# OPPO-Mente-Lab/PEA-Diffusion

Measured on AMD Instinct MI355X. Metric: training images/sec (SDXL 1024px bf16, adapter-only bwd), higher is better.
Workload: dtype bf16

## Files before the change

### include/pea_hip.h

```cpp
#ifndef PEA_HIP_H
#define PEA_HIP_H
#include <stdint.h>
#ifdef __cplusplus
extern "C" {
#endif

#define PEA_OK 0
#define PEA_E_INVALID (-1)
#define PEA_E_HIP (-2)
#define PEA_E_SHAPE (-3)
#define PEA_E_STATE (-4)
#define PEA_E_NOTFOUND (-5)
#define PEA_E_TIMEOUT (-6)

const char* pea_last_error(void);
int pea_version(void);
int pea_device_count(void);


int pea_op_gemm(const void* A, int lda, const void* W, int ldw, void* C, int ldc, int M, int N, int K, float alpha,
                const float* bias, const void* rowvec, int ldrv, int rows_per_batch, int act, void* preact,
                int ldpre, const void* res, int ldres, int out_f32, int accum_f32, void* stream);

int pea_op_gemm_qscale(const void* A, int lda, const void* W, int ldw, void* C, int ldc, int M, int N, int K, const float* bias,
// ... 176 lines not shown
int pea_unet_residual_info(void* unet, int i, int* C, int* H, int* W);
int pea_unet_set_residuals(void* unet, int n, const void* const* ptrs, int dtype, float scale, void* stream);
int pea_unet_set_inpaint_cond(void* unet, const float* mask, const float* masked_latents, int cond_batch, int latent_batch,
                              void* stream);
int pea_unet_clear_inpaint_cond(void* unet);
int pea_unet_set_freeu(void* unet, float s1, float s2, float b1, float b2, void* stream);
int pea_unet_clear_freeu(void* unet);
int pea_unet_ip_plan(const pea_unet_config* cfg, int n_tokens, int* n_layers, int* cols, long long* n_params);
int pea_unet_ip_create(void* unet, int n_tokens);
int pea_unet_ip_load_weight(void* unet, const char* key, const float* src, long long numel, void* stream);
int pea_unet_ip_set_tokens(void* unet, const float* tokens, void* stream);
int pea_unet_ip_set_scale(void* unet, float scale);
int pea_unet_ip_clear(void* unet);
int pea_unet_ip_destroy(void* unet);
int pea_unet_ip_export_kv(void* unet, float* out, long long* rows, int* cols, void* stream);
int pea_unet_ip_create_sets(void* unet, int n_sets, const int* n_tokens);
int pea_unet_ip_load_weight_set(void* unet, int set, const char* key, const float* src, long long numel, void* stream);
int pea_unet_ip_set_tokens_set(void* unet, int set, const float* tokens, void* stream);
int pea_unet_ip_set_scale_set(void* unet, int set, float scale);
int pea_unet_ip_clear_set(void* unet, int set);
int pea_unet_ip_set_layer_scales(void* unet, int set, const float* scales, int n_layers);
int pea_unet_ip_query_counts(void* unet, int* counts, int cap, int* n);
int pea_unet_ip_set_mask(void* unet, int set, int Sq, const float* mask, int Bm, void* stream);
int pea_unet_destroy(void* unet);

int pea_controlnet_create(const pea_unet_config* cfg, int B, int H, int W, int L, void** out);
int pea_controlnet_set_cond(void* cn, const float* image, void* stream);
int pea_controlnet_forward(void* cn, const float* x, const float* t, const void* ehs, int ehs_dtype, const void* text,
                           int text_dtype, const float* time_ids, void* stream);
int pea_controlnet_num_outputs(void* cn);
int pea_controlnet_output(void* cn, int i, void** ptr, int* C, int* H, int* W);
int pea_controlnet_export_nchw(void* cn, int i, float* dst, void* stream);

typedef struct pea_text_config {
  int vocab, max_pos, width, heads, layers, intermediate;
  int act;
  int flavor;
  int proj_dim;
  float eps;
  int pos_offset;
  long long eos_id;
  int rel_buckets;
  int rel_max_dist;
} pea_text_config;
int pea_text_create(const pea_text_config* cfg, int B, int L, void** out);
int pea_text_plan_attention(const pea_text_config* cfg, int B, int L, int* n_attn, int* n_prescaled);
int pea_text_forward(void* enc, const long long* ids, int hidden_index, float* hidden_out, float* pooled_out, void* stream);
int pea_text_rel_bias(void* enc, float* bias_out, void* stream);

typedef struct pea_vision_config {
  int image_size, patch_size, width, heads, layers, intermediate;
  int act;
  int proj_dim;
  float eps;
} pea_vision_config;
int pea_vision_create(const pea_vision_config* cfg, int B, void** out);
int pea_vision_plan(const pea_vision_config* cfg, int B, long long* n_params, int* n_tokens, int* n_attn);
int pea_vision_forward(void* enc, const float* pixels, int hidden_index, float* hidden_out, float* pooled_out, float* embeds_out,
                       void* stream);
typedef struct pea_resampler_config {
  int embed_dim, dim, heads, depth, n_queries, ff_inner, out_dim;
  float eps;
} pea_resampler_config;
int pea_resampler_create(const pea_resampler_config* cfg, int B, int S, void** out);
int pea_resampler_plan(const pea_resampler_config* cfg, int B, int S, long long* n_params, int* n_attn, int* n_prescaled);
int pea_resampler_plan_weight(const pea_resampler_config* cfg, int B, int S, int i, char* name, int name_len, long long* numel,
                              int* kind, int* d0, int* d1);
int pea_resampler_forward(void* resampler, const float* hidden, float* tokens_out, void* stream);
int pea_op_preprocess(const float* images, int B, int H, int W, float lo, float hi, int quantize, const int* y_first,
                      const int* y_count, const float* y_weights, int y_taps, const int* x_first, const int* x_count,
                      const float* x_weights, int x_taps, int size, int tile_h, int tile_w, int win_h, int win_w, float mean0,
                      float mean1, float mean2, float std0, float std1, float std2, float* out, void* stream);
int pea_op_patchify(const float* pixels, void* rows, int B, int S, int P, int kpad, void* stream);
int pea_op_clip_score(const float* image_embeds, const float* text_embeds, float* out, int B, int D, float w, int clamp,
                      void* stream);

int pea_vae_encoder_create(const pea_unet_config* cfg, int B, int H, int W, void** out);
int pea_vae_latent_shape(void* vae, int* C, int* H, int* W);
int pea_vae_encode(void* vae, const float* pixels, const float* noise, float scaling, float* moments, float* latents,
                   void* stream);
int pea_vae_decoder_create(const pea_unet_config* cfg, int B, int H, int W, void** out);
int pea_vae_decode(void* vae, const float* latents, float inv_scaling, float* image, void* stream);
int pea_unet_num_weights(void* unet);
int pea_unet_weight_info(void* unet, int i, char* name, int name_len, long long* numel, int* kind, int* d0, int* d1);
int pea_unet_load_weight(void* unet, const char* name, const float* src, long long numel, void* stream);
int pea_unet_load_weight_lora(void* unet, const char* name, const float* base, long long numel, int n_adapters,
                              const float* const* downs, const float* const* ups, const int* ranks, const float* scales,
                              void* stream);
int pea_unet_init_random(void* unet, unsigned long long seed, void* stream);
int pea_unet_share_weights(void* dst, void* src);
int pea_unet_forward(void* unet, const float* x, const float* t, const void* ehs, int ehs_dtype, const void* text,
                     int text_dtype, const float* time_ids, float* eps_out, void* stream);
int pea_unet_num_taps(void* unet);
int pea_unet_tap_name(void* unet, int k, char* name, int name_len);
int pea_unet_tap_info(void* unet, int k, void** data, void** grad, int* B, int* H, int* W, int* C);
int pea_unet_tap_export_nchw(void* unet, int k, int grad, float* out, void* stream);
int pea_unet_tap_layout(void* unet, int k);
int pea_unet_tap_import_grad_nchw(void* unet, int k, const float* src, void* stream);
int pea_unet_backward(void* unet, const float* deps, unsigned tap_seed_mask, void* stream);
int pea_unet_input_grads(void* unet, void** d_ehs, void** d_text);
int pea_unet_stacked_grad(void* unet, int which, float* out, long long* rows, int* cols, void* stream);
int pea_unet_stacked_layout(void* unet, int which, int i, char* name, int name_len, int* col_off, int* cols);
int pea_unet_memory(void* unet, long long* weight_bytes, long long* act_bytes, long long* grad_bytes, int* n_ops);
int pea_unet_release_activations(void* unet);

int pea_adapter_create(int in_dim, int out_dim, int hidden_dim, int out_dim1, int use_residual, void** out);
int pea_adapter_destroy(void* ad);
long long pea_adapter_num_params(void* ad);
int pea_adapter_bind(void* ad, float* flat_params);
int pea_adapter_prepare(void* ad, int batch, int L);
int pea_adapter_sync(void* ad, void* stream);
int pea_adapter_forward(void* ad, const void* enc, int dtype, float* pooled, float* tokens, void* stream);
int pea_adapter_backward(void* ad, const float* d_pooled, const float* d_tokens, float* grads, int accumulate,
                         void* stream);

int pea_trainer_create(void* adapter, void* student, void* teacher, float feat_weight, int nan_guard,
                       const float* alphas_cumprod, void** out);
int pea_trainer_destroy(void* tr);
int pea_train_step(void* tr, const float* latents, const float* noise, const long long* timesteps,
                   const float* enc, const float* enc_uncond, const unsigned char* prompt_mask,
                   const long long* zh_or_not, const float* teacher_ehs, const float* teacher_neg,
                   const float* teacher_pooled, const float* time_ids, float grad_scale, float* grads,
                   int accumulate, float* losses, void* stream);
int pea_trainer_set_option(void* tr, const char* name, int value);
int pea_trainer_backward_context(void* trainer, void** unet);
int pea_trainer_get_option(void* trainer, const char* name);
int pea_trainer_release_activations(void* trainer);
int pea_trainer_export(void* tr, int which, float* out, void* stream);

int pea_comm_unique_id(void* out128);
int pea_comm_init(int rank, int world, const void* unique_id128, void** comm_out);
int pea_comm_init_timeout(int rank, int world, const void* unique_id128, double timeout_s, void** comm_out);
int pea_comm_destroy(void* comm);
int pea_comm_world(void* comm);
int pea_comm_rank(void* comm);
int pea_allreduce_grads(void* comm, float* grads, long long n, void* compute_stream);
int pea_comm_join(void* comm, void* stream);
int pea_comm_last_ms(void* comm, float* ms);
int pea_comm_last_exposed_ms(void* comm, float* ms);
int pea_comm_broadcast(void* comm, float* buf, long long n, int root, void* stream);

void pea_prof_enable(int on);
void pea_prof_reset(void);
const char* pea_prof_family_name(int fam);
int pea_prof_dump(const char* path);
int pea_prof_report(int fam, double* ms, double* flops, double* bytes, long long* launches);
int pea_probe_mfma_peak(double seconds, int shape32, double* tflops, double* clock_mhz, void* stream);

void pea_debug_set_attn_tr(int v);
void pea_debug_set_attn_fused_bwd(int v);
void pea_debug_set_attn_xattn(int v);
void pea_debug_set_xattn_bwd_v2(int v);
void pea_debug_set_geglu_bwd_fused(int v);
void pea_debug_set_gemm_variant(int v);
int pea_debug_gemm_dispatch(int M, int N, int K, int mode, int rows_per_batch, int features, int cus, int forced);
int pea_debug_attn_dispatch(const int* q, int* out);
void pea_debug_set_gemm_debug(int v);
void pea_debug_set_gemm_prefetch(const void* p, long long bytes);

int pea_op_attention_fwd_regions(const void* Q, int ldq, const void* K, int ldk, const void* V, int ldv, void* O, int ldo, int B, int H,
                                 int Sq, int R, int Lr, const float* w, int Bw, float scale, int q_prescaled, void* stream);
int pea_unet_set_prompt_regions(void* unet, int R, int Sq, const float* w, int Bw, void* stream);
int pea_unet_clear_prompt_regions(void* unet);
int pea_debug_attn_regions_dispatch(const int* q, int* out);

int pea_op_attention_maps(const void* Q, int ldq, const void* K, int ldk, float* maps, int B, int H, int Sq, int Skv, float scale,
                          int q_prescaled, const int* kv_len, int accumulate, void* stream);
int pea_unet_enable_attention_maps(void* unet, const float* layer_on, int n_layers);
int pea_unet_reset_attention_maps(void* unet, void* stream);
int pea_unet_disable_attention_maps(void* unet);
int pea_unet_attention_maps(void* unet, int Sq, float** maps, long long* n_accumulated);
int pea_debug_attn_maps_dispatch(const int* q, int* out);

int pea_op_attention_fwd_edit(const void* Q, int ldq, const void* K, int ldk, const void* V, int ldv, void* O, int ldo, int B, int H,
                              int Sq, int Skv, const int* src, const void* Mt, int ldm, const float* c, const float* d, float scale,
                              int q_prescaled, void* stream);
int pea_unet_set_prompt_edit(void* unet, const int* src, const void* Mt, const float* cd, int T, int self_until, int self_max_tokens,
                             void* stream);
int pea_unet_set_prompt_edit_step(void* unet, int step);
int pea_unet_clear_prompt_edit(void* unet);
int pea_debug_attn_edit_dispatch(const int* q, int* out);

long long pea_op_attn_adain_scratch_bytes(int B, int H, int S);
int pea_op_attn_adain_coef(const void* Q, int ldq, const void* K, int ldk, int B, int H, int S, const int* ref, float scale,
                           int q_prescaled, int adain_queries, int adain_keys, float* coef, void* scratch, void* stream);
int pea_op_attention_fwd_shared(const void* Q, int ldq, const void* K, int ldk, const void* V, int ldv, void* O, int ldo, int B, int H,
                                int Sq, int Skv, const int* ref, const float* coef, float scale, int q_prescaled,
                                float shared_score_scale, float shared_score_shift, int nd, void* stream);
int pea_unet_set_style_aligned(void* unet, const int* ref, const float* layer_on, int n_layers, int adain_queries, int adain_keys,
                               float shared_score_scale, float shared_score_shift, void* stream);
int pea_unet_clear_style_aligned(void* unet);
int pea_unet_num_self_attention_layers(void* unet);
int pea_debug_attn_shared_dispatch(const int* q, int* out);

int pea_op_attention_colsum_groups(int B, int H, int Sq, int Skv);
int pea_op_attention_colsum(const void* Q, int ldq, const void* K, int ldk, const float* lse, float* part, int B, int H, int Sq, int Skv,
                            float scale, int q_prescaled, void* stream);
int pea_debug_attn_colsum_dispatch(const int* q, int* out);
int pea_op_sag_degrade(const float* latents, const float* eps, const float* part, int G, int map_h, int map_w, const int* iy,
                       const int* ix, float* out, int B, int C, int H, int W, float c_x, float c_e, float o_b, float o_e, void* stream);
int pea_op_cfg_sag_combine(const float* eps, const float* eps_deg, float* out, int B, long long per, int cfg, float guidance_scale,
                           float sag_scale, void* stream);
int pea_unet_enable_sag(void* unet, int layer, int first_sample, int n_samples);
int pea_unet_disable_sag(void* unet);
int pea_unet_sag_colsum(void* unet, float** part, int* G, int* S);

int pea_op_query_blur(void* Q, int ld, int col0, int n, int h, int w, int C, const float* Mh, const float* Mw, void* stream);
int pea_op_query_blur_lds_bytes(int h, int w);
int pea_op_attn_identity(const void* V, int ldv, int col0, void* O, int ldo, long long rows, int C, void* stream);
int pea_op_cfg_pag_combine(const float* eps, float* out, int B, long long per, int cfg, float guidance_scale, float pag_scale,
                           float guidance_rescale, void* workspace, void* stream);
int pea_unet_set_attn_perturb(void* unet, int mode, int first_sample, const float* layer_on, int n_layers, int n_grids,
                              const int* grid_h, const int* grid_w, const float* tables, void* stream);
int pea_unet_clear_attn_perturb(void* unet);

#ifdef __cplusplus
}
#endif
#endif
```

### pea_diffusion_amd/csrc/norm.hip

```cpp
#include "pea_kernels.h"
#ifndef PEA_LN_WT
#define PEA_LN_WT 1
#endif

#define GN_MAX_GROUPS 64

template <int BWD>
__global__ void gn_stats_kernel(const bf16* __restrict__ x, const bf16* __restrict__ dy,
                                const float* __restrict__ gamma, const float* __restrict__ beta,
                                const float* __restrict__ stats, float* __restrict__ partial, int HW, int C,
                                int groups, int pix_per_block, int silu) {
  extern __shared__ __attribute__((aligned(16))) char gsm[];
  const int nchunk = C / 8;
  const int ppb = blockDim.x / nchunk;
  const int tid = threadIdx.x;
  const int b = blockIdx.y;
  const int cpg = C / groups;
  float* tsum = (float*)gsm;
  float* csum = tsum + ppb * nchunk * 16;
  const int ck = tid % nchunk, pl = tid / nchunk;
  float s1[8], s2[8];
#pragma unroll
  for (int j = 0; j < 8; ++j) s1[j] = s2[j] = 0.f;
  if (pl < ppb) {
// ... 278 lines not shown
#pragma unroll
      for (int j = 0; j < VEC; ++j) {
        const float d = GN_X(i, j) - GN_SEL(j, mean0, mean1);
        if (GW == 2 && hi[j]) s[1] += d * d; else s[0] += d * d;
      }
    if (!act) s[0] = s[1] = 0.f;
    double q[2];
    gn_block_sum<GW>(s, red, q);
    gn_pin(xr);
    const float rstd0 = (float)(1.0 / sqrt(q[0] / count + (double)eps));
    const float rstd1 = GW == 2 ? (float)(1.0 / sqrt(q[1] / count + (double)eps)) : 0.f;
    if (tid == 0) {
      stats[sg * 2] = mean0; stats[sg * 2 + 1] = rstd0;
      if (GW == 2) { stats[sg * 2 + 2] = mean1; stats[sg * 2 + 3] = rstd1; }
    }
    if (!act) return;
    float sc[VEC], sh[VEC];
#pragma unroll
    for (int j = 0; j < VEC; ++j) {
      sc[j] = GN_SEL(j, rstd0, rstd1) * gamma[c0 + j];
      sh[j] = beta[c0 + j] - GN_SEL(j, mean0, mean1) * sc[j];
    }
#pragma unroll
    for (int i = 0; i < NPIX; ++i) {
      uint32_t o[W];
#pragma unroll
      for (int w = 0; w < W; ++w) {
        float v0 = GN_X(i, 2 * w) * sc[2 * w] + sh[2 * w], v1 = GN_X(i, 2 * w + 1) * sc[2 * w + 1] + sh[2 * w + 1];
        if (SILU) { v0 = siluf_(v0); v1 = siluf_(v1); }
        o[w] = gn_pack(v0, v1);
      }
      gn_store<W>(out + sbase + i * istep + toff, o);
    }
  } else {
    const float mean0 = stats[sg * 2], rstd0 = stats[sg * 2 + 1];
    const float mean1 = GW == 2 ? stats[sg * 2 + 2] : 0.f, rstd1 = GW == 2 ? stats[sg * 2 + 3] : 0.f;
    float gm[VEC], bt[VEC];
#pragma unroll
    for (int j = 0; j < VEC; ++j) { gm[j] = gamma[c0 + j]; bt[j] = beta[c0 + j]; }
    float s[2 * GW];
#pragma unroll
    for (int k = 0; k < 2 * GW; ++k) s[k] = 0.f;
#pragma unroll
    for (int i = 0; i < NPIX; ++i) {
#pragma unroll
      for (int j = 0; j < VEC; ++j) {
        const float xh = (GN_X(i, j) - GN_SEL(j, mean0, mean1)) * GN_SEL(j, rstd0, rstd1);
        float d = GN_D(i, j);
        if (SILU) d *= silu_grad(xh * gm[j] + bt[j]);
        d *= gm[j];
        if (GW == 2 && hi[j]) { s[1] += d; s[3] += d * xh; } else { s[0] += d; s[GW] += d * xh; }
      }
      if (i + 1 < NPIX) gn_chain<W>(s[GW], xr[i + 1], dr[i + 1]);
    }
    if (!act) {
#pragma unroll
      for (int k = 0; k < 2 * GW; ++k) s[k] = 0.f;
    }
    double r[2 * GW];
    gn_block_sum<2 * GW>(s, red, r);
    gn_pin(xr);
    gn_pin(dr);
    if (!act) return;
    const float S10 = (float)(r[0] / count), S20 = (float)(r[GW] / count);
    const float S11 = GW == 2 ? (float)(r[1] / count) : 0.f, S21 = GW == 2 ? (float)(r[2 * GW - 1] / count) : 0.f;
#pragma unroll
    for (int i = 0; i < NPIX; ++i) {
      uint32_t o[W];
      if (add) gn_load<W>(o, add + sbase + i * istep + toff);
#pragma unroll
      for (int w = 0; w < W; ++w) {
        float rr[2];
#pragma unroll
        for (int h = 0; h < 2; ++h) {
          const int j = 2 * w + h;
          const float rs = GN_SEL(j, rstd0, rstd1);
          const float xh = (GN_X(i, j) - GN_SEL(j, mean0, mean1)) * rs;
          float d = GN_D(i, j);
          if (SILU) d *= silu_grad(xh * gm[j] + bt[j]);
          d *= gm[j];
          rr[h] = rs * (d - GN_SEL(j, S10, S11) - xh * GN_SEL(j, S20, S21));
          if (add) rr[h] += h ? gn_hi(o[w]) : gn_lo(o[w]);
        }
        o[w] = gn_pack(rr[0], rr[1]);
      }
      if (i + 1 < NPIX) {
        float dep = __builtin_bit_cast(float, o[W - 1]);
        gn_chain<W>(dep, xr[i + 1], dr[i + 1]);
        o[W - 1] = __builtin_bit_cast(uint32_t, dep);
      }
      gn_store<W>(out + sbase + i * istep + toff, o);
    }
  }
#undef GN_X
#undef GN_D
#undef GN_SEL
}

struct GnFused { int vec, npix, gw, threads, ppb; };
static bool gn_fused_geometry(int HW, int C, int groups, int bwd, GnFused* f) {
  static const bool off = getenv("PEA_GN_UNFUSED") != nullptr;
  if (off) return false;
  const int cpg = C / groups;
  if (cpg % 8 == 0) { f->vec = 8; f->gw = 1; }
  else if (cpg % 4 == 0) { f->vec = 4; f->gw = 1; }
  else if (cpg % 2 == 0 && groups % 2 == 0) { f->vec = 4; f->gw = 2; }
  else return false;
  const int nvec = f->gw * cpg / f->vec;
  for (int npix = 8; npix <= 32; npix *= 2) {
    if (HW % npix) continue;
    const int regs = npix * f->vec / 2 * (1 + bwd);
    if (regs > 128) return false;
    const int maxt = regs > 64 ? 640 : 1024;
    const int thr = nvec * (HW / npix);
    if (thr > maxt) continue;
    f->npix = npix; f->ppb = HW / npix; f->threads = (thr + 63) / 64 * 64;
    return true;
  }
  return false;
}

template <int BWD>
static void gn_fused_launch(const GnFused& f, int blocks, hipStream_t s, const bf16* x, const bf16* dy, const float* gamma,
                            const float* beta, float* stats, bf16* out, const bf16* add, int HW, int C, int groups, float eps,
                            int silu) {
#define GN_S(V, N, G, S) hipLaunchKernelGGL((gn_fused_kernel<V, N, BWD, G, S>), dim3(blocks), dim3(f.threads), 0, s, x, dy, gamma, beta, \
                                            stats, out, add, HW, C, groups, f.ppb, eps)
#define GN_G(V, N, G) do { if (silu) GN_S(V, N, G, 1); else GN_S(V, N, G, 0); } while (0)
#define GN_F(V, N) do { if (f.gw == 2) GN_G(V, N, 2); else GN_G(V, N, 1); } while (0)
  if (f.vec == 8) {
    switch (f.npix) { case 8: GN_F(8, 8); break; case 16: GN_F(8, 16); break; default: GN_F(8, 32); break; }
  } else {
    switch (f.npix) { case 8: GN_F(4, 8); break; case 16: GN_F(4, 16); break; default: GN_F(4, 32); break; }
  }
#undef GN_S
#undef GN_G
#undef GN_F
}

static int gn_geometry(int HW, int C, int* threads, int* ppblk, int* nblk, size_t* lds) {
  const int nchunk = C / 8;
  if (nchunk > 1024) return -1;
  int ppb = 256 / nchunk;
  if (ppb < 1) ppb = 1;
  *threads = nchunk * ppb;
  int per = ppb * 16;
  if (per > HW) per = HW;
  *ppblk = per;
  *nblk = cdiv(HW, per);
  *lds = (size_t)(*threads) * 16 * 4 + (size_t)2 * C * 4;
  return 0;
}

size_t groupnorm_scratch_bytes(int B, int HW, int C, int groups) {
  int threads, ppblk, nblk;
  size_t lds;
  if (gn_geometry(HW, C, &threads, &ppblk, &nblk, &lds)) return 0;
  return ((size_t)B * nblk * groups * 2 + (size_t)B * groups * 2) * sizeof(float) + 256;
}

int launch_groupnorm_fwd(const bf16* x, const float* gamma, const float* beta, bf16* y, float* stats,
                         double* scratch, int B, int HW, int C, int groups, float eps, int silu, hipStream_t s) {
  SHAPECHK(C % 8 == 0 && C % groups == 0 && groups <= GN_MAX_GROUPS, "groupnorm: C=%d groups=%d", C, groups);
  int threads, ppblk, nblk;
  size_t lds;
  SHAPECHK(gn_geometry(HW, C, &threads, &ppblk, &nblk, &lds) == 0, "groupnorm: C=%d too wide", C);
  SHAPECHK(threads >= groups, "groupnorm: C=%d too narrow for %d groups", C, groups);
  float* partial = (float*)scratch;
  PROF_BEGIN(4, 0.0, 2.0 * 2.0 * B * (double)HW * C, s);
  GnFused f;
  if (gn_fused_geometry(HW, C, groups, 0, &f)) {
    gn_fused_launch<0>(f, B * (groups / f.gw), s, x, nullptr, gamma, beta, stats, y, nullptr, HW, C, groups, eps, silu);
    PROF_END(s);
    HIPCHK(hipGetLastError());
    return PEA_OK;
  }
  hipLaunchKernelGGL(gn_stats_kernel<0>, dim3(nblk, B), dim3(threads), lds, s, x, nullptr, nullptr, nullptr, nullptr,
                     partial, HW, C, groups, ppblk, 0);
  hipLaunchKernelGGL(gn_finalize_kernel, dim3(B * groups), dim3(64), 0, s, partial, stats, B * groups, groups, nblk,
                     (double)HW * (C / groups), eps, 0);
  hipLaunchKernelGGL(gn_apply_kernel, dim3(nblk, B), dim3(threads), 0, s, x, gamma, beta, stats, y, HW, C, groups,
                     silu, ppblk);
  PROF_END(s);
  HIPCHK(hipGetLastError());
  return PEA_OK;
}

int launch_groupnorm_bwd(const bf16* x, const bf16* dy, const float* gamma, const float* beta, const float* stats,
                         bf16* dx, double* scratch, int B, int HW, int C, int groups, int silu, const bf16* add,
                         hipStream_t s) {
  SHAPECHK(C % 8 == 0 && C % groups == 0 && groups <= GN_MAX_GROUPS, "groupnorm: C=%d groups=%d", C, groups);
  int threads, ppblk, nblk;
  size_t lds;
  SHAPECHK(gn_geometry(HW, C, &threads, &ppblk, &nblk, &lds) == 0, "groupnorm: C=%d too wide", C);
  SHAPECHK(threads >= groups, "groupnorm: C=%d too narrow for %d groups", C, groups);
  float* partial = (float*)scratch;
  float* sums = partial + (size_t)B * nblk * groups * 2;
  PROF_BEGIN(4, 0.0, 2.0 * (add ? 4.0 : 3.0) * B * (double)HW * C, s);
  GnFused f;
  if (gn_fused_geometry(HW, C, groups, 1, &f)) {
    gn_fused_launch<1>(f, B * (groups / f.gw), s, x, dy, gamma, beta, const_cast<float*>(stats), dx, add, HW, C, groups, 0.f, silu);
    PROF_END(s);
    HIPCHK(hipGetLastError());
    return PEA_OK;
  }
  hipLaunchKernelGGL(gn_stats_kernel<1>, dim3(nblk, B), dim3(threads), lds, s, x, dy, gamma, beta, stats, partial, HW,
                     C, groups, ppblk, silu);
  hipLaunchKernelGGL(gn_finalize_kernel, dim3(B * groups), dim3(64), 0, s, partial, sums, B * groups, groups, nblk,
                     (double)HW * (C / groups), 0.f, 1);
  hipLaunchKernelGGL(gn_bwd_apply_kernel, dim3(nblk, B), dim3(threads), 0, s, x, dy, gamma, beta, stats, sums, dx, HW,
                     C, groups, silu, add, ppblk);
  PROF_END(s);
  HIPCHK(hipGetLastError());
  return PEA_OK;
}

#define LN_MAXCH 8

#define LN_NR 2
template <int NCH, bool STATS_ONLY = false>
__global__ __launch_bounds__(256) void ln_fwd_kernel(const bf16* __restrict__ x, const float* __restrict__ gamma,
                                                     const float* __restrict__ beta, bf16* __restrict__ y,
                                                     float* __restrict__ stats, int R, int C, float eps) {
  const int lane = threadIdx.x & 63;
  const int row0 = (blockIdx.x * 4 + (threadIdx.x >> 6)) * LN_NR;
  if (row0 >= R) return;
  const int nchunk = C / 8;
  bf16x8 v[LN_NR][NCH];
#pragma unroll
  for (int r = 0; r < LN_NR; ++r) {
    const int row = min(row0 + r, R - 1);
#pragma unroll
    for (int i = 0; i < NCH; ++i) {
      const int ck = min(lane + 64 * i, nchunk - 1);
      v[r][i] = *(const bf16x8*)(x + (long long)row * C + ck * 8);
    }
  }
  f32x4 g0[STATS_ONLY ? 1 : NCH], g1[STATS_ONLY ? 1 : NCH], b0[STATS_ONLY ? 1 : NCH], b1[STATS_ONLY ? 1 : NCH];
  if constexpr (!STATS_ONLY) {
#pragma unroll
    for (int i = 0; i < NCH; ++i) {
      const int ck = min(lane + 64 * i, nchunk - 1);
      g0[i] = *(const f32x4*)(gamma + ck * 8); g1[i] = *(const f32x4*)(gamma + ck * 8 + 4);
      b0[i] = *(const f32x4*)(beta + ck * 8); b1[i] = *(const f32x4*)(beta + ck * 8 + 4);
    }
  }
  float mean[LN_NR], rstd[LN_NR];
#pragma unroll
  for (int r = 0; r < LN_NR; ++r) {
    float s = 0.f;
#pragma unroll
    for (int i = 0; i < NCH; ++i)
      if (lane + 64 * i < nchunk)
#pragma unroll
        for (int j = 0; j < 8; ++j) s += (float)v[r][i][j];
    mean[r] = wave_sum(s) / (float)C;
    float q = 0.f;
#pragma unroll
    for (int i = 0; i < NCH; ++i)
      if (lane + 64 * i < nchunk)
#pragma unroll
        for (int j = 0; j < 8; ++j) {
          const float d = (float)v[r][i][j] - mean[r];
          q += d * d;
        }
    rstd[r] = rsqrtf(wave_sum(q) / (float)C + eps);
    if (stats && lane == 0 && row0 + r < R) {
      stats[2 * (long long)(row0 + r)] = mean[r];
      stats[2 * (long long)(row0 + r) + 1] = rstd[r];
    }
  }
  if constexpr (STATS_ONLY) return;
#pragma unroll
  for (int i = 0; i < NCH; ++i) {
    const int ck = lane + 64 * i;
    if (ck < nchunk) {
#pragma unroll
      for (int r = 0; r < LN_NR; ++r) {
        if (row0 + r >= R) break;
        bf16x8 o;
#pragma unroll
        for (int j = 0; j < 4; ++j) {
          o[j] = (bf16)(((float)v[r][i][j] - mean[r]) * rstd[r] * g0[STATS_ONLY ? 0 : i][j] + b0[STATS_ONLY ? 0 : i][j]);
          o[4 + j] = (bf16)(((float)v[r][i][4 + j] - mean[r]) * rstd[r] * g1[STATS_ONLY ? 0 : i][j] + b1[STATS_ONLY ? 0 : i][j]);
        }
        store16<PEA_LN_WT != 0>(y + (long long)(row0 + r) * C + ck * 8, o);
      }
    }
  }
}

template <int NCH>
__global__ __launch_bounds__(256) void ln_bwd_kernel(const bf16* __restrict__ x, const bf16* __restrict__ dy,
                                                     const float* __restrict__ gamma,
                                                     const float* __restrict__ stats, bf16* dx,
                                                     float* __restrict__ dgamma, float* __restrict__ dbeta, int R,
                                                     int C, const bf16* add) {
  const int lane = threadIdx.x & 63;
  const int row0 = (blockIdx.x * 4 + (threadIdx.x >> 6)) * LN_NR;
  if (row0 >= R) return;
  const int nchunk = C / 8;
  bf16x8 xv[LN_NR][NCH], dv[LN_NR][NCH], av[LN_NR][NCH];
#pragma unroll
  for (int r = 0; r < LN_NR; ++r) {
    const int row = min(row0 + r, R - 1);
#pragma unroll
    for (int i = 0; i < NCH; ++i) {
      const int ck = min(lane + 64 * i, nchunk - 1);
      xv[r][i] = *(const bf16x8*)(x + (long long)row * C + ck * 8);
      dv[r][i] = *(const bf16x8*)(dy + (long long)row * C + ck * 8);
      if (add) av[r][i] = *(const bf16x8*)(add + (long long)row * C + ck * 8);
    }
  }
  f32x4 g0[NCH], g1[NCH];
#pragma unroll
  for (int i = 0; i < NCH; ++i) {
    const int ck = min(lane + 64 * i, nchunk - 1);
    g0[i] = *(const f32x4*)(gamma + ck * 8); g1[i] = *(const f32x4*)(gamma + ck * 8 + 4);
  }
  float2 st[LN_NR];
#pragma unroll
  for (int r = 0; r < LN_NR; ++r) st[r] = *(const float2*)(stats + 2 * (long long)min(row0 + r, R - 1));
  __builtin_amdgcn_sched_barrier(0);
#pragma unroll
  for (int r = 0; r < LN_NR; ++r) {
    const float mean = st[r].x, rstd = st[r].y;
    float s1 = 0.f, s2 = 0.f;
#pragma unroll
    for (int i = 0; i < NCH; ++i)
      if (lane + 64 * i < nchunk)
#pragma unroll
        for (int j = 0; j < 8; ++j) {
          const float xh = ((float)xv[r][i][j] - mean) * rstd;
          const float d = (float)dv[r][i][j] * (j < 4 ? g0[i][j] : g1[i][j - 4]);
          s1 += d;
          s2 += d * xh;
        }
    s1 = wave_sum(s1) / (float)C;
    s2 = wave_sum(s2) / (float)C;
    if (row0 + r >= R) break;
#pragma unroll
    for (int i = 0; i < NCH; ++i) {
      const int ck = lane + 64 * i;
      if (ck < nchunk) {
        bf16x8 o;
#pragma unroll
        for (int j = 0; j < 8; ++j) {
          const float xh = ((float)xv[r][i][j] - mean) * rstd;
          float rr = rstd * ((float)dv[r][i][j] * (j < 4 ? g0[i][j] : g1[i][j - 4]) - s1 - xh * s2);
          if (add) rr += (float)av[r][i][j];
          o[j] = (bf16)rr;
        }
        store16<PEA_LN_WT != 0>(dx + (long long)(row0 + r) * C + ck * 8, o);
      }
// ... 190 lines not shown
```

Before: 39.22.

## Add split-pixel two-kernel GroupNorm path for paired-group backward shapes

Adds a GroupNorm path that splits each group's pixels across many blocks. A sums kernel writes per-piece partial statistics, and an apply kernel reduces those partials and normalises its own piece with values kept in registers. It is picked by default only for backward shapes where the fused one-block-per-group kernel handles two groups per block with 32 pixels per thread, aiming to raise parallelism over a kernel with too few blocks. The cost is a second launch and reading x and dy twice, and the path can be forced or disabled through a debug setter.

```diff
diff --git a/include/pea_hip.h b/include/pea_hip.h
--- a/include/pea_hip.h
+++ b/include/pea_hip.h
@@ -352,6 +352,7 @@
 void pea_debug_set_attn_xattn(int v);
 void pea_debug_set_xattn_bwd_v2(int v);
 void pea_debug_set_geglu_bwd_fused(int v);
+void pea_debug_set_gn_path(int v);
 void pea_debug_set_gemm_variant(int v);
 int pea_debug_gemm_dispatch(int M, int N, int K, int mode, int rows_per_batch, int features, int cus, int forced);
 int pea_debug_attn_dispatch(const int* q, int* out);
diff --git a/pea_diffusion_amd/csrc/norm.hip b/pea_diffusion_amd/csrc/norm.hip
--- a/pea_diffusion_amd/csrc/norm.hip
+++ b/pea_diffusion_amd/csrc/norm.hip
@@ -454,6 +454,281 @@
   return 0;
 }
 
+#define GNS_T 256
+#define GNS_NPIX 8
+
+struct GnSplit { int vec, gw, ppb, S, piece; };
+
+template <int VEC, int GW>
+struct GnSplitIdx {
+  int b, pc, gs, vk, c0, p1, ch;
+  bool act;
+  long long sbase;
+  int pix[GNS_NPIX];
+  bool ok[GNS_NPIX];
+  __device__ __forceinline__ GnSplitIdx(int HW, int C, int groups, int ppb, int S, int piece) {
+    const int cpg = C / groups, nset = groups / GW, span = GW * cpg, nvec = span / VEC;
+    const int total = gridDim.x, bid = blockIdx.x;
+    const int idx = (total % 8 == 0) ? (bid % 8) * (total / 8) + bid / 8 : bid;
+    gs = idx % nset;
+    const int t = idx / nset;
+    b = t / S; pc = t - b * S;
+    const int tid = threadIdx.x, pl = tid / nvec;
+    vk = tid - pl * nvec;
+    act = pl < ppb;
+    c0 = gs * span + vk * VEC;
+    const int p0 = pc * piece;
+    p1 = min(p0 + piece, HW);
+    sbase = (long long)b * HW * C;
+    ch = C;
+#pragma unroll
+    for (int i = 0; i < GNS_NPIX; ++i) {
+      const int p = p0 + pl + i * ppb;
+      ok[i] = act && p < p1;
+      pix[i] = min(p, p1 - 1);
+    }
+  }
+  __device__ __forceinline__ long long off(int i) const { return sbase + (long long)pix[i] * ch + c0; }
+};
+
+template <int VEC, int BWD, int GW, int SILU>
+__global__ __launch_bounds__(GNS_T) void gn_split_sums_kernel(const bf16* __restrict__ x, const bf16* __restrict__ dy,
+                                                              const float* __restrict__ gamma, const float* __restrict__ beta,
+                                                              const float* __restrict__ stats, float* __restrict__ partial,
+                                                              int HW, int C, int groups, int ppb, int S, int piece) {
+  constexpr int W = VEC / 2;
+  __shared__ double red[16][4];
+  const GnSplitIdx<VEC, GW> ix(HW, C, groups, ppb, S, piece);
+  const int cpg = C / groups;
+  uint32_t xr[GNS_NPIX][W];
+  uint32_t dr[BWD ? GNS_NPIX : 1][W];
+#pragma unroll
+  for (int i = 0; i < GNS_NPIX; ++i) {
+    gn_load<W>(xr[i], x + ix.off(i));
+    if (BWD) gn_load<W>(dr[i], dy + ix.off(i));
+  }
+  bool hi[VEC];
+#pragma unroll
+  for (int j = 0; j < VEC; ++j) hi[j] = GW == 2 && (ix.vk * VEC + j) >= cpg;
+#define GN_X(i, j) (((j) & 1) ? gn_hi(xr[i][(j) >> 1]) : gn_lo(xr[i][(j) >> 1]))
+#define GN_D(i, j) (((j) & 1) ? gn_hi(dr[i][(j) >> 1]) : gn_lo(dr[i][(j) >> 1]))
+#define GN_SEL(j, a0, a1) ((GW == 2 && hi[j]) ? (a1) : (a0))
+  float s[2 * GW];
+#pragma unroll
+  for (int k = 0; k < 2 * GW; ++k) s[k] = 0.f;
+  if (!BWD) {
+#pragma unroll
+    for (int i = 0; i < GNS_NPIX; ++i)
+#pragma unroll
+      for (int j = 0; j < VEC; ++j) {
+        const float v = ix.ok[i] ? GN_X(i, j) : 0.f;
+        if (GW == 2 && hi[j]) { s[1] += v; s[2 * GW - 1] += v * v; } else { s[0] += v; s[GW] += v * v; }
+      }
+  } else {
+    const long long sg = (long long)ix.b * groups + ix.gs * GW;
+    const float mean0 = stats[sg * 2], rstd0 = stats[sg * 2 + 1];
+    const float mean1 = GW == 2 ? stats[sg * 2 + 2] : 0.f, rstd1 = GW == 2 ? stats[sg * 2 + 3] : 0.f;
+    float gm[VEC], bt[VEC];
+#pragma unroll
+    for (int j = 0; j < VEC; j += 4) {
+      const f32x4 g4 = *(const f32x4*)(gamma + ix.c0 + j), b4 = *(const f32x4*)(beta + ix.c0 + j);
+#pragma unroll
+      for (int q = 0; q < 4; ++q) { gm[j + q] = g4[q]; bt[j + q] = b4[q]; }
+    }
+#pragma unroll
+    for (int i = 0; i < GNS_NPIX; ++i)
+#pragma unroll
+      for (int j = 0; j < VEC; ++j) {
+        const float xh = (GN_X(i, j) - GN_SEL(j, mean0, mean1)) * GN_SEL(j, rstd0, rstd1);
+        float d = GN_D(i, j);
+        if (SILU) d *= silu_grad(xh * gm[j] + bt[j]);
+        d *= gm[j];
+        if (!ix.ok[i]) d = 0.f;
+        if (GW == 2 && hi[j]) { s[1] += d; s[2 * GW - 1] += d * xh; } else { s[0] += d; s[GW] += d * xh; }
+      }
+  }
+  double r[2 * GW];
+  gn_block_sum<2 * GW>(s, red, r);
+  if (threadIdx.x < GW) {
+    const int h = threadIdx.x;
+    float* o = partial + (((long long)ix.b * S + ix.pc) * groups + ix.gs * GW + h) * 2;
+    o[0] = (float)((GW == 2 && h) ? r[1] : r[0]);
+    o[1] = (float)((GW == 2 && h) ? r[2 * GW - 1] : r[GW]);
+  }
+#undef GN_X
+#undef GN_D
+#undef GN_SEL
+}
+
+template <int VEC, int BWD, int GW, int SILU>
+__global__ __launch_bounds__(GNS_T) void gn_split_apply_kernel(const bf16* __restrict__ x, const bf16* __restrict__ dy,
+                                                               const float* __restrict__ gamma, const float* __restrict__ beta,
+                                                               float* stats, const float* __restrict__ partial, bf16* out,
+                                                               const bf16* add, int HW, int C, int groups, int ppb, int S,
+                                                               int piece, float eps) {
+  constexpr int W = VEC / 2;
+  const GnSplitIdx<VEC, GW> ix(HW, C, groups, ppb, S, piece);
+  const int cpg = C / groups;
+  uint32_t xr[GNS_NPIX][W];
+  uint32_t dr[BWD ? GNS_NPIX : 1][W];
+  uint32_t ar[BWD ? GNS_NPIX : 1][W];
+#pragma unroll
+  for (int i = 0; i < GNS_NPIX; ++i) {
+    gn_load<W>(xr[i], x + ix.off(i));
+    if (BWD) {
+      gn_load<W>(dr[i], dy + ix.off(i));
+      if (add) gn_load<W>(ar[i], add + ix.off(i));
+    }
+  }
+  float gm[VEC], bt[VEC];
+#pragma unroll
+  for (int j = 0; j < VEC; j += 4) {
+    const f32x4 g4 = *(const f32x4*)(gamma + ix.c0 + j), b4 = *(const f32x4*)(beta + ix.c0 + j);
+#pragma unroll
+    for (int q = 0; q < 4; ++q) { gm[j + q] = g4[q]; bt[j + q] = b4[q]; }
+  }
+  const long long sg = (long long)ix.b * groups + ix.gs * GW;
+  float mean[2] = {0.f, 0.f}, rstd[2] = {0.f, 0.f};
+  if (BWD) {
+#pragma unroll
+    for (int h = 0; h < GW; ++h) { mean[h] = stats[(sg + h) * 2]; rstd[h] = stats[(sg + h) * 2 + 1]; }
+  }
+  const int lane = threadIdx.x & 63;
+  double a[2 * GW];
+#pragma unroll
+  for (int k = 0; k < 2 * GW; ++k) a[k] = 0.0;
+  for (int k = lane; k < S; k += 64) {
+    const float* p = partial + (((long long)ix.b * S + k) * groups + ix.gs * GW) * 2;
+#pragma unroll
+    for (int h = 0; h < GW; ++h) { a[h] += (double)p[2 * h]; a[GW + h] += (double)p[2 * h + 1]; }
+  }
+#pragma unroll
+  for (int o = 32; o > 0; o >>= 1)
+#pragma unroll
+    for (int k = 0; k < 2 * GW; ++k) a[k] += __shfl_xor(a[k], o, 64);
+  const double count = (double)HW * cpg;
+  bool hi[VEC];
+#pragma unroll
+  for (int j = 0; j < VEC; ++j) hi[j] = GW == 2 && (ix.vk * VEC + j) >= cpg;
+#define GN_X(i, j) (((j) & 1) ? gn_hi(xr[i][(j) >> 1]) : gn_lo(xr[i][(j) >> 1]))
+#define GN_D(i, j) (((j) & 1) ? gn_hi(dr[i][(j) >> 1]) : gn_lo(dr[i][(j) >> 1]))
+#define GN_SEL(j, a0, a1) ((GW == 2 && hi[j]) ? (a1) : (a0))
+  if (!BWD) {
+#pragma unroll
+    for (int h = 0; h < GW; ++h) {
+      const double m = a[h] / count;
+      double var = a[GW + h] / count - m * m;
+      if (var < 0) var = 0;
+      mean[h] = (float)m;
+      rstd[h] = (float)(1.0 / sqrt(var + (double)eps));
+    }
+    if (ix.pc == 0 && threadIdx.x < GW) {
+      const int h = threadIdx.x;
+      stats[(sg + h) * 2] = h ? mean[1] : mean[0];
+      stats[(sg + h) * 2 + 1] = h ? rstd[1] : rstd[0];
+    }
+    float sc[VEC], sh[VEC];
+#pragma unroll
+    for (int j = 0; j < VEC; ++j) {
+      sc[j] = GN_SEL(j, rstd[0], rstd[1]) * gm[j];
+      sh[j] = bt[j] - GN_SEL(j, mean[0], mean[1]) * sc[j];
+    }
+#pragma unroll
+    for (int i = 0; i < GNS_NPIX; ++i) {
+      uint32_t o[W];
+#pragma unroll
+      for (int w = 0; w < W; ++w) {
+        float v0 = GN_X(i, 2 * w) * sc[2 * w] + sh[2 * w], v1 = GN_X(i, 2 * w + 1) * sc[2 * w + 1] + sh[2 * w + 1];
+        if (SILU) { v0 = siluf_(v0); v1 = siluf_(v1); }
+        o[w] = gn_pack(v0, v1);
+      }
+      if (ix.ok[i]) gn_store<W>(out + ix.off(i), o);
+    }
+  } else {
+    float S1[2] = {0.f, 0.f}, S2[2] = {0.f, 0.f};
+#pragma unroll
+    for (int h = 0; h < GW; ++h) { S1[h] = (float)(a[h] / count); S2[h] = (float)(a[GW + h] / count); }
+#pragma unroll
+    for (int i = 0; i < GNS_NPIX; ++i) {
+      uint32_t o[W];
+#pragma unroll
+      for (int w = 0; w < W; ++w) {
+        float rr[2];
+#pragma unroll
+        for (int h = 0; h < 2; ++h) {
+          const int j = 2 * w + h;
+          const float rs = GN_SEL(j, rstd[0], rstd[1]);
+          const float xh = (GN_X(i, j) - GN_SEL(j, mean[0], mean[1])) * rs;
+          float d = GN_D(i, j);
+          if (SILU) d *= silu_grad(xh * gm[j] + bt[j]);
+          d *= gm[j];
+          rr[h] = rs * (d - GN_SEL(j, S1[0], S1[1]) - xh * GN_SEL(j, S2[0], S2[1]));
+          if (add) rr[h] += h ? gn_hi(ar[i][w]) : gn_lo(ar[i][w]);
+        }
+        o[w] = gn_pack(rr[0], rr[1]);
+      }
+      if (ix.ok[i]) gn_store<W>(out + ix.off(i), o);
+    }
+  }
+#undef GN_X
+#undef GN_D
+#undef GN_SEL
+}
+
+static bool gn_split_geometry(int HW, int C, int groups, GnSplit* f) {
+  const int cpg = C / groups;
+  if (cpg % 8 == 0) { f->vec = 8; f->gw = 1; }
+  else if (cpg % 4 == 0) { f->vec = 4; f->gw = 1; }
+  else if (cpg % 2 == 0 && groups % 2 == 0) { f->vec = 4; f->gw = 2; }
+  else return false;
+  const int nvec = f->gw * cpg / f->vec;
+  if (nvec > GNS_T) return false;
+  f->ppb = GNS_T / nvec;
+  f->S = cdiv(HW, f->ppb * GNS_NPIX);
+  f->piece = cdiv(HW, f->S);
+  int threads, ppblk, nblk;
+  size_t lds;
+  if (gn_geometry(HW, C, &threads, &ppblk, &nblk, &lds)) return false;
+  return f->S <= nblk;
+}
+
+template <int BWD>
+static void gn_split_launch(const GnSplit& f, int B, hipStream_t s, const bf16* x, const bf16* dy, const float* gamma,
+                            const float* beta, float* stats, float* partial, bf16* out, const bf16* add, int HW, int C,
+                            int groups, float eps, int silu) {
+  const int blocks = B * f.S * (groups / f.gw);
+#define GN_S(V, G, S_)                                                                                                          \
+  do {                                                                                                                          \
+    hipLaunchKernelGGL((gn_split_sums_kernel<V, BWD, G, S_>), dim3(blocks), dim3(GNS_T), 0, s, x, dy, gamma, beta, stats,       \
+                       partial, HW, C, groups, f.ppb, f.S, f.piece);                                                            \
+    hipLaunchKernelGGL((gn_split_apply_kernel<V, BWD, G, S_>), dim3(blocks), dim3(GNS_T), 0, s, x, dy, gamma, beta, stats,      \
+                       partial, out, add, HW, C, groups, f.ppb, f.S, f.piece, eps);                                             \
+  } while (0)
+#define GN_G(V, G) do { if (silu) GN_S(V, G, 1); else GN_S(V, G, 0); } while (0)
+  if (f.vec == 8) GN_G(8, 1); else if (f.gw == 2) GN_G(4, 2); else GN_G(4, 1);
+#undef GN_S
+#undef GN_G
+}
+
+enum { GN_PATH_ONE = 1, GN_PATH_SPLIT = 2, GN_PATH_GENERAL = 3 };
+static int g_gn_path = 0;
+extern "C" void pea_debug_set_gn_path(int v) { g_gn_path = v; }
+
+static bool gn_split_wins(const GnFused& f, int bwd) {
+  return bwd && f.gw == 2 && f.npix == 32;
+}
+
+static int gn_choose(int HW, int C, int groups, int bwd, GnFused* f, GnSplit* sp) {
+  const bool one = gn_fused_geometry(HW, C, groups, bwd, f);
+  const bool split = gn_split_geometry(HW, C, groups, sp);
+  static const bool unfused = getenv("PEA_GN_UNFUSED") != nullptr;
+  if (unfused || g_gn_path == GN_PATH_GENERAL) return GN_PATH_GENERAL;
+  if (g_gn_path == GN_PATH_ONE) return one ? GN_PATH_ONE : GN_PATH_GENERAL;
+  if (g_gn_path == GN_PATH_SPLIT) return split ? GN_PATH_SPLIT : GN_PATH_GENERAL;
+  if (one && split && gn_split_wins(*f, bwd)) return GN_PATH_SPLIT;
+  return one ? GN_PATH_ONE : GN_PATH_GENERAL;
+}
+
 size_t groupnorm_scratch_bytes(int B, int HW, int C, int groups) {
   int threads, ppblk, nblk;
   size_t lds;
@@ -469,10 +744,21 @@
   SHAPECHK(gn_geometry(HW, C, &threads, &ppblk, &nblk, &lds) == 0, "groupnorm: C=%d too wide", C);
   SHAPECHK(threads >= groups, "groupnorm: C=%d too narrow for %d groups", C, groups);
   float* partial = (float*)scratch;
+  GnFused f;
+  GnSplit sp;
+  const int path = gn_choose(HW, C, groups, 0, &f, &sp);
+  if (path == GN_PATH_SPLIT)
+    SHAPECHK(((size_t)B * sp.S * groups * 2) * sizeof(float) <= groupnorm_scratch_bytes(B, HW, C, groups),
+             "groupnorm: %d pieces do not fit the scratch", sp.S);
   PROF_BEGIN(4, 0.0, 2.0 * 2.0 * B * (double)HW * C, s);
-  GnFused f;
-  if (gn_fused_geometry(HW, C, groups, 0, &f)) {
+  if (path == GN_PATH_ONE) {
     gn_fused_launch<0>(f, B * (groups / f.gw), s, x, nullptr, gamma, beta, stats, y, nullptr, HW, C, groups, eps, silu);
+    PROF_END(s);
+    HIPCHK(hipGetLastError());
+    return PEA_OK;
+  }
+  if (path == GN_PATH_SPLIT) {
+    gn_split_launch<0>(sp, B, s, x, nullptr, gamma, beta, stats, partial, y, nullptr, HW, C, groups, eps, silu);
     PROF_END(s);
     HIPCHK(hipGetLastError());
     return PEA_OK;
@@ -498,10 +784,21 @@
   SHAPECHK(threads >= groups, "groupnorm: C=%d too narrow for %d groups", C, groups);
   float* partial = (float*)scratch;
   float* sums = partial + (size_t)B * nblk * groups * 2;
+  GnFused f;
+  GnSplit sp;
+  const int path = gn_choose(HW, C, groups, 1, &f, &sp);
+  if (path == GN_PATH_SPLIT)
+    SHAPECHK(((size_t)B * sp.S * groups * 2) * sizeof(float) <= groupnorm_scratch_bytes(B, HW, C, groups),
+             "groupnorm: %d pieces do not fit the scratch", sp.S);
   PROF_BEGIN(4, 0.0, 2.0 * (add ? 4.0 : 3.0) * B * (double)HW * C, s);
-  GnFused f;
-  if (gn_fused_geometry(HW, C, groups, 1, &f)) {
+  if (path == GN_PATH_ONE) {
     gn_fused_launch<1>(f, B * (groups / f.gw), s, x, dy, gamma, beta, const_cast<float*>(stats), dx, add, HW, C, groups, 0.f, silu);
+    PROF_END(s);
+    HIPCHK(hipGetLastError());
+    return PEA_OK;
+  }
+  if (path == GN_PATH_SPLIT) {
+    gn_split_launch<1>(sp, B, s, x, dy, gamma, beta, const_cast<float*>(stats), partial, dx, add, HW, C, groups, 0.f, silu);
     PROF_END(s);
     HIPCHK(hipGetLastError());
     return PEA_OK;
```

After: 39.21 (median of 2 runs). No clear change (-0.0%).
